# youshyee/CoSA

Measured on AMD Instinct MI355X. Metric: training images/sec at 448x448 ViT-B, higher is better.
Workload: dtype bf16; 1 GPU; VOC12 21-class, ViT-B/16 bf16, batch 16/GPU x 448x448, teacher 3 scales x 2 flips + student fwd/bwd + cam2mask x2 + 5 losses + AdamW + EMA; global_batch=16, parallelism=dp1, defer_groups=1, grid_policy=full grid

## Files before the change

### cosa_amd/csrc/gemm_kernels.hip

```cpp
#include "kernels.hpp"
#include "op16.hpp"
#include "c8.hpp"
#include "c4.hpp"
#include <cstdlib>

namespace cosa {
namespace {

typedef float f32x4 __attribute__((ext_vector_type(4)));

constexpr int BM = 128, BN = 128, BK = 64;
constexpr int TILE_BYTES = 128 * BK * 2;
constexpr int STAGE_BYTES = 2 * TILE_BYTES;
constexpr int CT_LD = 272;

enum { EPI_BIAS = 0, EPI_GELU = 1, EPI_RESIDUAL = 2 };

__device__ __forceinline__ float gelu_erf(float x)
{
    const float z = __builtin_fabsf(x) * 0.70710678118654752f;
    const float t = __builtin_amdgcn_rcpf(__builtin_fmaf(0.3275911f, z, 1.0f));
    float p = __builtin_fmaf(1.061405429f, t, -1.453152027f);
    p = __builtin_fmaf(p, t, 1.421413741f);
    p = __builtin_fmaf(p, t, -0.284496736f);
    p = __builtin_fmaf(p, t, 0.254829592f);
    p = p * t;
    const float e = __builtin_amdgcn_exp2f(-z * z * 1.4426950408889634f);
    const float erf_abs = __builtin_fmaf(-p, e, 1.0f);
    const float erfx = __builtin_copysignf(erf_abs, x);
    return 0.5f * x * (1.0f + erfx);
}

#define COSA_SPLIT_OPAQUE(a, b) asm volatile("" : "+v"(a), "+v"(b))

typedef __attribute__((address_space(3))) void lds_void;
typedef const __attribute__((address_space(1))) void gbl_void;

__device__ __forceinline__ void stage_tile(const op16 *__restrict__ src, int row0, int nrows, int ld, int k0,
                                           unsigned char *lds_tile, int wave, int lane)
{
#pragma unroll
    for (int i = 0; i < 4; i++) {
        const int q = wave * 4 + i;
        const int row = 8 * q + (lane >> 3);
        const int s = (lane & 7) ^ (row & 7);
        int grow = row0 + row;
        grow = grow < nrows ? grow : nrows - 1;
        const op16 *g = src + (size_t)grow * ld + k0 + s * 8;
        __builtin_amdgcn_global_load_lds((gbl_void *)g, (lds_void *)(lds_tile + q * 1024), 16, 0, 0);
    }
}

struct SplitGeom { int Kp; };
__device__ __forceinline__ int split_tile_x(int kt, int Kp) { return kt <= 2 * Kp ? kt : kt - 2 * Kp - 1; }
__device__ __forceinline__ int split_tile_w(int kt, int Kp) { return kt < Kp ? kt : (kt < 2 * Kp ? kt - Kp : (kt == 2 * Kp ? kt : kt - Kp - 1)); }

__device__ __forceinline__ bool c8_is_f8(int kt, int Kp) { return kt > Kp; }
__device__ __forceinline__ int c8_tile_x(int kt, int Kp) { return kt < Kp ? kt : (kt == Kp ? 2 * Kp : kt - 1); }
__device__ __forceinline__ int c8_tile_w(int kt, int Kp)
{
    const int Kh = Kp >> 1;
    return kt < Kp ? kt : (kt == Kp ? 2 * Kp : (kt <= Kp + Kh ? kt + Kh - 1 : kt - Kh - 1));
}
typedef int c8_i32x8 __attribute__((ext_vector_type(8)));
typedef int c8_i32x4 __attribute__((ext_vector_type(4)));
__device__ __forceinline__ c8_i32x8 c8_cat(op16x8 lo, op16x8 hi)
{
    return __builtin_shufflevector(__builtin_bit_cast(c8_i32x4, lo), __builtin_bit_cast(c8_i32x4, hi), 0, 1, 2, 3, 4, 5, 6, 7);
}
constexpr int kC8ScaleW = 0x7f7f7f7f;
constexpr int kC8ScaleX = 0x74747474;
#define COSA_MFMA_C8(a8, b8, c) __builtin_amdgcn_mfma_scale_f32_16x16x128_f8f6f4(a8, b8, c, 1, 1, 0, kC8ScaleW, 0, kC8ScaleX)

template <int OA, int OB>
__device__ __forceinline__ f32x4 mfma_c4(c8_i32x8 a4, c8_i32x8 b4, f32x4 c, int sa, int sb)
{
    return __builtin_amdgcn_mfma_scale_f32_16x16x128_f8f6f4(a4, b4, c, 4, 4, OA, sa, OB, sb);
}
__device__ __forceinline__ c8_i32x8 c4_op(op16x8 v)
{
    const c8_i32x4 t = __builtin_bit_cast(c8_i32x4, v);
    return (c8_i32x8){t[0], t[1], t[2], t[3], 0, 0, 0, 0};
}
__device__ __forceinline__ float c4_max4(float v)
{
    const unsigned u = __builtin_bit_cast(unsigned, v);
    const auto a = __builtin_amdgcn_permlane16_swap(u, u, false, false);
    const unsigned m = a[0] > a[1] ? a[0] : a[1];
    const auto b = __builtin_amdgcn_permlane32_swap(m, m, false, false);
    return __builtin_bit_cast(float, b[0] > b[1] ? b[0] : b[1]);
}
constexpr int kC4ScaleLds = 16384;
constexpr int kStageLdsC4 = 16384, kStageLds = 32768;

template <int EPI, int SPLIT = 0>
__global__ __launch_bounds__(256, 2) void gemm_bf16_kernel(const op16 *__restrict__ X, const op16 *__restrict__ W,
                                                          const op16 *__restrict__ bias, const float *__restrict__ R,
                                                          void *__restrict__ Yv, int M, int N, int K, int tiles_m, int tiles_n,
                                                          int ld, int ldy, void *__restrict__ Y2v, int tail_o0 = -1)
{
    static_assert(SPLIT < 3 || (SPLIT == 3 && EPI == EPI_RESIDUAL), "fp16c8 operands: residual epilogue (tail mode) only; fp16c4: not supported here");
    extern __shared__ __attribute__((aligned(16))) unsigned char smem[];
    const int tid = threadIdx.x, wave = tid >> 6, lane = tid & 63;
    int m0, n0;
    if (tail_o0 >= 0) {
        const int ntl = tiles_m * tiles_n, cq = ntl >> 3, cr = ntl & 7;
        const int o = tail_o0 + ((int)blockIdx.x >> 2), sub = blockIdx.x & 3;
        const int xcd = o & 7, idx = o >> 3;
        const int t = (xcd < cr ? xcd * (cq + 1) : cr * (cq + 1) + (xcd - cr) * cq) + idx;
        const int tm = t / tiles_n;
        m0 = tm * 256 + (sub >> 1) * BM;
        n0 = (t - tm * tiles_n) * 256 + (sub & 1) * BN;
        if (m0 >= M) return;
    } else {
        const int nwg = tiles_m * tiles_n;
        int wg = blockIdx.x;
        {
            const int q = nwg >> 3, r = nwg & 7, xcd = wg & 7, idx = wg >> 3;
            wg = (xcd < r ? xcd * (q + 1) : r * (q + 1) + (xcd - r) * q) + idx;
        }
        const int tm = wg / tiles_n, tn = wg - tm * tiles_n;
        m0 = tm * BM;
        n0 = tn * BN;
    }
    const int wr = wave >> 1, wc = wave & 1;

    f32x4 acc[4][4];
    const bool tail = tail_o0 >= 0;
#pragma unroll
    for (int i = 0; i < 4; i++)
#pragma unroll
        for (int j = 0; j < 4; j++) {
            acc[i][j] = (f32x4){0.f, 0.f, 0.f, 0.f};
            if (tail) {
                const int nl = (wave >> 1) * 64 + 16 * i + 4 * (lane >> 4), ml = (wave & 1) * 64 + 16 * j + (lane & 15);
                if (EPI == EPI_RESIDUAL) {
                    if (m0 + ml < M) acc[i][j] = *reinterpret_cast<const f32x4 *>(R + (size_t)(m0 + ml) * N + n0 + nl);
                } else {
#pragma unroll
                    for (int r = 0; r < 4; r++) acc[i][j][r] = (float)bias[n0 + nl + r];
                }
            }
        }

    const int Kp = K / BK;
    const int nk = SPLIT == 1 ? 3 * Kp + 1 : (SPLIT == 3 ? 2 * Kp + 1 : Kp);
    auto tile_x = [&](int kt) { return SPLIT == 1 ? split_tile_x(kt, Kp) : (SPLIT == 3 ? c8_tile_x(kt, Kp) : kt); };
    auto tile_w = [&](int kt) { return SPLIT == 1 ? split_tile_w(kt, Kp) : (SPLIT == 3 ? c8_tile_w(kt, Kp) : kt); };
    stage_tile(W, n0, N, ld, 0, smem, wave, lane);
    stage_tile(X, m0, M, ld, 0, smem + TILE_BYTES, wave, lane);
    asm volatile("s_waitcnt vmcnt(0)" ::: "memory");
    __syncthreads();

    const int frow = lane & 15, fq = lane >> 4;
    for (int kt = 0; kt < nk; kt++) {
        unsigned char *cur = smem + (kt & 1) * STAGE_BYTES;
        unsigned char *nxt = smem + ((kt + 1) & 1) * STAGE_BYTES;
        if (kt + 1 < nk) {
            stage_tile(W, n0, N, ld, tile_w(kt + 1) * BK, nxt, wave, lane);
            stage_tile(X, m0, M, ld, tile_x(kt + 1) * BK, nxt + TILE_BYTES, wave, lane);
        }
        const unsigned char *At = cur + (wr * 64) * 128;
        const unsigned char *Bt = cur + TILE_BYTES + (wc * 64) * 128;
        if (SPLIT == 3 && kt > Kp) {
            op16x8 a2[4][2], b2[4][2];
#pragma unroll
            for (int i = 0; i < 4; i++) {
                const int row = i * 16 + frow;
#pragma unroll
                for (int ks = 0; ks < 2; ks++) {
                    const int slot = ((fq + 4 * ks) ^ (row & 7)) << 4;
                    a2[i][ks] = *reinterpret_cast<const op16x8 *>(At + row * 128 + slot);
                    b2[i][ks] = *reinterpret_cast<const op16x8 *>(Bt + row * 128 + slot);
                }
            }
#pragma unroll
            for (int i = 0; i < 4; i++) {
                const c8_i32x8 a8 = c8_cat(a2[i][0], a2[i][1]);
#pragma unroll
                for (int j = 0; j < 4; j++) acc[i][j] = COSA_MFMA_C8(a8, c8_cat(b2[j][0], b2[j][1]), acc[i][j]);
            }
        } else
#pragma unroll
        for (int ks = 0; ks < 2; ks++) {
            op16x8 a[4], b[4];
#pragma unroll
            for (int i = 0; i < 4; i++) {
                const int row = i * 16 + frow;
                const int slot = ((fq + 4 * ks) ^ (row & 7)) << 4;
                a[i] = *reinterpret_cast<const op16x8 *>(At + row * 128 + slot);
                b[i] = *reinterpret_cast<const op16x8 *>(Bt + row * 128 + slot);
            }
#pragma unroll
            for (int i = 0; i < 4; i++)
#pragma unroll
                for (int j = 0; j < 4; j++)
                    acc[i][j] = COSA_MFMA_16x16x32(a[i], b[j], acc[i][j], 0, 0, 0);
        }
        asm volatile("s_waitcnt vmcnt(0)" ::: "memory");
        __syncthreads();
    }

    unsigned char *Ct = smem;
#pragma unroll
    for (int i = 0; i < 4; i++) {
        const int nl = wr * 64 + 16 * i + 4 * fq;
        float bv[4];
#pragma unroll
        for (int r = 0; r < 4; r++) bv[r] = (tail && EPI != EPI_RESIDUAL) ? 0.0f : (float)bias[n0 + nl + r];
#pragma unroll
        for (int j = 0; j < 4; j++) {
            const int ml = wc * 64 + 16 * j + frow;
            if (EPI == EPI_RESIDUAL) {
                f32x4 v;
#pragma unroll
                for (int r = 0; r < 4; r++) v[r] = acc[i][j][r] + bv[r];
                *reinterpret_cast<f32x4 *>(Ct + ml * (BN * 4 + 16) + nl * 4) = v;
            } else {
                op16x4 v, vlo;
#pragma unroll
                for (int r = 0; r < 4; r++) {
                    float t = acc[i][j][r] + bv[r];
                    if (SPLIT == 2) {
                        v[r] = (op16)t;
                        vlo[r] = (op16)gelu_erf(t);
                    } else {
                        if (EPI == EPI_GELU) t = gelu_erf(t);
                        if (SPLIT) asm volatile("" : "+v"(t));
                        v[r] = (op16)t;
                        if (SPLIT) vlo[r] = (op16)(t - (float)v[r]);
                    }
                }
                *reinterpret_cast<op16x4 *>(Ct + ml * CT_LD + nl * 2) = v;
                if (SPLIT) *reinterpret_cast<op16x4 *>(Ct + BM * CT_LD + ml * CT_LD + nl * 2) = vlo;
            }
        }
    }
    __syncthreads();
    if (EPI == EPI_RESIDUAL) {
        float *Y = static_cast<float *>(Yv);
#pragma unroll
        for (int c = tid; c < BM * 32; c += 256) {
            const int ml = c >> 5, s = c & 31;
            if (m0 + ml < M) {
                const f32x4 v = *reinterpret_cast<const f32x4 *>(Ct + ml * (BN * 4 + 16) + s * 16);
                const size_t o = (size_t)(m0 + ml) * N + n0 + s * 4;
                if (tail) {
                    *reinterpret_cast<f32x4 *>(Y + o) = v;
                } else {
                    const f32x4 rv = *reinterpret_cast<const f32x4 *>(R + o);
                    *reinterpret_cast<f32x4 *>(Y + o) = v + rv;
                }
            }
        }
    } else {
        op16 *Y = static_cast<op16 *>(Yv);
#pragma unroll
        for (int c = tid; c < BM * 16; c += 256) {
            const int ml = c >> 4, s = c & 15;
            if (m0 + ml < M) {
                *reinterpret_cast<uint4 *>(Y + (size_t)(m0 + ml) * ldy + n0 + s * 8) =
                    *reinterpret_cast<const uint4 *>(Ct + ml * CT_LD + s * 16);
                if (SPLIT == 1)
                    *reinterpret_cast<uint4 *>(Y + (size_t)(m0 + ml) * ldy + N + n0 + s * 8) =
                        *reinterpret_cast<const uint4 *>(Ct + BM * CT_LD + ml * CT_LD + s * 16);
                if (SPLIT == 2)
                    *reinterpret_cast<uint4 *>(static_cast<op16 *>(Y2v) + (size_t)(m0 + ml) * ldy + n0 + s * 8) =
                        *reinterpret_cast<const uint4 *>(Ct + BM * CT_LD + ml * CT_LD + s * 16);
            }
        }
    }
}


constexpr int V5_HALF = 16384;
constexpr int V5_BUF = 4 * V5_HALF;
constexpr size_t kLdsBytesV5 = 2 * V5_BUF;

#define V5_FENCE() __builtin_amdgcn_sched_barrier(0)
#define V5_BARRIER()                          \
    do {                                      \
        V5_FENCE();                           \
        __builtin_amdgcn_s_barrier();         \
        V5_FENCE();                           \
    } while (0)

typedef unsigned u32x2 __attribute__((ext_vector_type(2)));
typedef unsigned u32x4 __attribute__((ext_vector_type(4)));

template <int EPI, int SPLIT = 0, int FR = 4>
__global__ __launch_bounds__(512, 1) void gemm_bf16_v6_kernel(const op16 *__restrict__ X, const op16 *__restrict__ W,
                                                             const op16 *__restrict__ bias, const float *__restrict__ R,
                                                             void *__restrict__ Yv, int M, int N, int K, int tiles_m, int tiles_n,
                                                             unsigned long long *__restrict__ stamps, int ld, int ldy, void *__restrict__ Y2v, int ntiles_run,
                                                             const unsigned char *__restrict__ xsc, const unsigned char *__restrict__ wsc, unsigned char *__restrict__ ysc)
{
    if (stamps && threadIdx.x == 0) atomicMin(&stamps[2 * (blockIdx.x & 63)], __builtin_amdgcn_s_memrealtime());
    constexpr bool RES = EPI == EPI_RESIDUAL;
    constexpr int ES = RES ? 4 : 2;
    constexpr int FL = 0x00020000;
    static_assert(FR == 4 || (FR == 3 && SPLIT == 0), "FR: 16-feature fragments per wave and W half (tile width 64 FR)");
// ... 992 lines not shown
    for (int i = 0; i < PER; i++) {
        const float a = v[i].x - mean, c = v[i].y - mean, d = v[i].z - mean, e = v[i].w - mean;
        q += a * a + c * c + d * d + e * e;
    }
#pragma unroll
    for (int o = 32; o > 0; o >>= 1) q += __shfl_xor(q, o, 64);
    const float rstd = rsqrtf(q * (1.0f / D) + eps);
#pragma unroll
    for (int i = 0; i < PER; i++) {
        const int c0 = (lane + 64 * i) * 4;
        const op16x4 gg = *reinterpret_cast<const op16x4 *>(g + c0);
        const op16x4 bb = *reinterpret_cast<const op16x4 *>(b + c0);
        float o0 = (v[i].x - mean) * rstd * (float)gg[0] + (float)bb[0];
        float o1 = (v[i].y - mean) * rstd * (float)gg[1] + (float)bb[1];
        float o2 = (v[i].z - mean) * rstd * (float)gg[2] + (float)bb[2];
        float o3 = (v[i].w - mean) * rstd * (float)gg[3] + (float)bb[3];
        if (y) {
            op16x4 ov;
            ov[0] = (op16)o0; ov[1] = (op16)o1; ov[2] = (op16)o2; ov[3] = (op16)o3;
            *reinterpret_cast<op16x4 *>(y + (size_t)row * D + c0) = ov;
        }
        if (y32) *reinterpret_cast<float4 *>(y32 + (size_t)row * D + c0) = make_float4(o0, o1, o2, o3);
    }
}

}
}

using namespace cosa;

#if COSA_OP_F16
#define cosa_gemm_set_stamp_slot cosa_gemm_set_stamp_slot_f16
#define cosa_gemm_set_variant cosa_gemm_set_variant_f16
#define cosa_gemm_set_grid_policy cosa_gemm_set_grid_policy_f16
#define cosa_gemm_bf16 cosa_gemm_f16
#define cosa_gemm_bf16x3 cosa_gemm_f16x3
#define cosa_layernorm cosa_layernorm_f16
#define cosa_gemm_wgrad_bf16 cosa_gemm_wgrad_f16
#define cosa_conv3x3_dilated_wgrad cosa_conv3x3_dilated_wgrad_f16
#define cosa_conv3x3_dilated_nhwc cosa_conv3x3_dilated_nhwc_f16
#endif

#include <type_traits>

static size_t cosa_c4_scale_bytes_(int rows, int K) { return (size_t)((rows + 255) / 256) * (size_t)(K / 128) * 2048; }
static unsigned long long *g_gemm_stamp_slot = nullptr;
extern "C" void cosa_gemm_set_stamp_slot(void *slot) { g_gemm_stamp_slot = static_cast<unsigned long long *>(slot); }
namespace {
struct ClearSlot { ~ClearSlot() { g_gemm_stamp_slot = nullptr; } };
}

static int g_gemm_balanced_grid = 0;
static int g_gemm_variant = 0;
extern "C" void cosa_gemm_set_variant(int v) { g_gemm_variant = v; }
extern "C" void cosa_gemm_set_grid_policy(int balanced) { g_gemm_balanced_grid = balanced; }

template <auto Kernel>
static int max_dynamic_lds_once(int bytes)
{
    static bool done = false;
    if (!done) {
        COSA_HIP_CHECK(hipFuncSetAttribute((const void *)Kernel, hipFuncAttributeMaxDynamicSharedMemorySize, bytes));
        done = true;
    }
    return COSA_OK;
}

template <class F>
static int with_epilogue(int epilogue, F &&f)
{
    if (epilogue == EPI_BIAS) return f(std::integral_constant<int, EPI_BIAS>{});
    if (epilogue == EPI_GELU) return f(std::integral_constant<int, EPI_GELU>{});
    return f(std::integral_constant<int, EPI_RESIDUAL>{});
}

template <class... A>
static int check_gemm_args(const char *who, bool operands, const char *operands_what, int epilogue, const float *residual, bool shape_ok,
                           const char *shape_fmt, A... shape_args)
{
    COSA_REQUIRE(operands, "%s: %s", who, operands_what);
    COSA_REQUIRE(shape_ok, shape_fmt, shape_args...);
    COSA_REQUIRE(epilogue >= 0 && epilogue <= 2, "%s: unknown epilogue", who);
    COSA_REQUIRE(epilogue != EPI_RESIDUAL || residual, "%s: residual epilogue needs the residual pointer", who);
    return COSA_OK;
}

constexpr size_t kReach = 0x7fffffffull;
static bool fits_persistent(int M, int N, int ld) { return (size_t)(M + 256) * ld * 2 < kReach && (size_t)N * ld * 2 < kReach; }
static bool fits_persistent_x3(int M, int N, int ld) { return (size_t)(M + 256) * ld * 2 < kReach * 8 && (size_t)N * ld * 2 < kReach; }
static bool fits_panels(int N, int ld, int ldy) { return (size_t)256 * ld * 2 < kReach && (size_t)N * ld * 2 < kReach && (size_t)256 * ldy * 4 < kReach; }

constexpr int small_lds_bytes(int split)
{
    return ((split == 1 || split == 2) && 2 * BM * CT_LD > (int)kLdsBytes) ? 2 * BM * CT_LD : (int)kLdsBytes;
}


template <int EPI, int SPLIT>
static int launch_small(const op16 *x, const op16 *w, const op16 *b, const float *residual, void *Y, void *Y2, int M, int N, int K, int ld, int ldy,
                        hipStream_t st, int first_job = -1, int njobs = 0)
{
    constexpr int lds_bytes = small_lds_bytes(SPLIT);
    if (int rc = max_dynamic_lds_once<gemm_bf16_kernel<EPI, SPLIT>>(lds_bytes)) return rc;
    const bool tail = first_job >= 0;
    const int tiles_m = tail ? (M + 255) / 256 : (M + BM - 1) / BM, tiles_n = tail ? N / 256 : N / BN;
    hipLaunchKernelGGL((gemm_bf16_kernel<EPI, SPLIT>), dim3(tail ? 4 * njobs : tiles_m * tiles_n), dim3(256), lds_bytes, st, x, w, b, residual, Y,
                       M, N, K, tiles_m, tiles_n, ld ? ld : K, ldy ? ldy : N, Y2, first_job);
    COSA_LAUNCH_CHECK();
    return COSA_OK;
}

static int persistent_jobs(int ntiles)
{
    constexpr int tail_max = 48;
    const int rem = ntiles % 256, rounds_up = (ntiles + 255) / 256;
    if (ntiles > 256 && rem != 0 && rem <= tail_max && (256 - rem) * 10 > 256 * rounds_up) return ntiles - rem;
    return ntiles;
}

template <int EPI, int SPLIT = 0, int FR = 4>
static int launch_v6(const op16 *x, const op16 *w, const op16 *b, const float *residual, void *Y, int M, int N, int K, hipStream_t st,
                     int ld = 0, int ldy = 0, void *Y2 = nullptr, const unsigned char *xsc = nullptr, const unsigned char *wsc = nullptr,
                     unsigned char *ysc = nullptr)
{
    constexpr size_t lds_bytes = kLdsBytesV5 + (SPLIT == 4 ? kC4ScaleLds + kStageLdsC4 : kStageLds);
    if (int rc = max_dynamic_lds_once<gemm_bf16_v6_kernel<EPI, SPLIT, FR>>((int)lds_bytes)) return rc;
    const int tiles_m = (M + 255) / 256, tiles_n = N / (64 * FR);
    const int ntiles = tiles_m * tiles_n;
    const int grid = ntiles < 256 ? ntiles : 256;
    constexpr bool can_tail = FR == 4 && (SPLIT == 0 || SPLIT == 1 || (SPLIT == 3 && EPI == EPI_RESIDUAL));
    const int run = can_tail ? persistent_jobs(ntiles) : ntiles;
    const bool balanced = g_gemm_balanced_grid != 0;
    int grid_b = grid;
    if (balanced && run > 256 && M < 40000) {
        const int rounds = (run + 255) / 256;
        grid_b = ((run + rounds - 1) / rounds + 7) / 8 * 8;
        grid_b = grid_b > 256 ? 256 : grid_b;
    }
    hipLaunchKernelGGL((gemm_bf16_v6_kernel<EPI, SPLIT, FR>), dim3(grid_b), dim3(512), lds_bytes, st, x, w, b, residual, Y, M, N, K, tiles_m, tiles_n,
                       g_gemm_stamp_slot, ld ? ld : K, ldy ? ldy : N, Y2, run, xsc, wsc, ysc);
    g_gemm_stamp_slot = nullptr;
    COSA_LAUNCH_CHECK();
    if constexpr (can_tail) {
        if (run < ntiles) return launch_small<EPI, SPLIT>(x, w, b, residual, Y, nullptr, M, N, K, ld, ldy, st, run, ntiles - run);
    }
    return COSA_OK;
}

extern "C" int cosa_gemm_bf16(const void *X, const void *W, const void *bias, const float *residual, void *Y,
                              int M, int N, int K, int epilogue, void *stream)
{
    ClearSlot clear_slot_;
    const bool positive = M > 0 && N > 0 && K > 0;
    if (int rc = check_gemm_args("cosa_gemm_bf16", X && W && bias && Y, "null pointer", epilogue, residual, positive && N % BN == 0 && K % BK == 0,
                                 positive ? "cosa_gemm_bf16: N must be a multiple of 128 and K of 64 (got N=%d K=%d)" : "cosa_gemm_bf16: bad shape", N, K))
        return rc;
    hipStream_t st = as_stream(stream);
    const op16 *x = static_cast<const op16 *>(X), *w = static_cast<const op16 *>(W), *b = static_cast<const op16 *>(bias);
    const bool fits_v5 = N % 256 == 0 && M >= 256 && fits_persistent(M, N, K);
    constexpr int big_m = 4096;
    const bool fits_v6 = fits_v5 && K >= 128 && (epilogue != EPI_RESIDUAL || g_gemm_variant == 6 || g_gemm_variant == 9 || g_gemm_variant == 0);
    if (fits_v6 && N % 192 == 0 && (g_gemm_variant == 9 || (g_gemm_variant == 0 && M >= big_m))) {
        constexpr int wide_max = 48;
        const long tm = (M + 255) / 256, n4 = tm * (N / 256), n3 = tm * (N / 192);
        const double r4 = (n4 > 256 && n4 % 256 != 0 && n4 % 256 <= wide_max) ? (double)(n4 / 256) + 0.1 : (double)((n4 + 255) / 256);
        const double r3 = 0.78 * (double)((n3 + 255) / 256);
        if (g_gemm_variant == 9 || r3 < r4 - 0.05)
            return with_epilogue(epilogue, [&](auto e) { return launch_v6<decltype(e)::value, 0, 3>(x, w, b, residual, Y, M, N, K, st); });
    }
    if (fits_v6 && (g_gemm_variant == 6 || (g_gemm_variant == 0 && M >= big_m)))
        return with_epilogue(epilogue, [&](auto e) { return launch_v6<decltype(e)::value>(x, w, b, residual, Y, M, N, K, st); });
    return with_epilogue(epilogue, [&](auto e) { return launch_small<decltype(e)::value, 0>(x, w, b, residual, Y, nullptr, M, N, K, K, N, st); });
}

extern "C" int cosa_gemm_bf16x3(const void *Xs, const void *Ws, const void *zeros, const float *residual, void *Y,
                                int M, int N, int K, int epilogue, int ldy, void *stream)
// ... 208 lines not shown
```

### cosa_amd/nn_ops.py

```python
import contextlib
import ctypes
import math
import os
import time
import weakref

import torch
import torch.nn.functional as F
from torch.autograd import Function

from . import _C


_flops = {}


_reference_ops = None


def reference_op(name, what, *args, **kw):
    if _reference_ops is None:
        raise _C.CosaError(f"{what}: no HIP kernel covers this shape / dtype and cosa_amd has no second backend "
                           "(torch reference operators exist only in the test-suite: tests/torch_reference.py)")
    return _reference_ops[name](*args, **kw)
# ... 86 lines not shown
    def backward(ctx, dout):
        qkv, out, lse = ctx.saved_tensors
        H = ctx.H
        B, N, _ = qkv.shape
        dout = dout.contiguous()
        dqkv = torch.empty_like(qkv)
        L = _C.lib()
        ws = _C.workspace(L.cosa_attn_bwd_workspace_bytes(B, N, H), qkv.device, "attn_bwd")
        with _C.profiled("attn_bwd"):
            _C.check(L.cosa_attn_bwd(_C.ptr(qkv), _C.ptr(out), _C.ptr(dout), _C.ptr(lse), _C.ptr(dqkv), B, N, H, 64, 0.125,
                                     _C.ptr(ws), ws.numel(), _C.stream_ptr()), "cosa_attn_bwd")
        _flops["attn_bwd"] = _flops.get("attn_bwd", 0) + 10.0 * B * H * N * N * 64
        return dqkv, None


def attention(qkv, H):
    if qkv.dtype == torch.bfloat16:
        return FusedAttention.apply(qkv, H)
    return reference_op("attention", f"attention on {qkv.dtype} operands", qkv, H)


EPI_BIAS, EPI_GELU, EPI_RESIDUAL = 0, 1, 2


def gemm_bf16(x, w, b, epilogue=EPI_BIAS, residual=None, out=None):
    M, K = x.shape
    N = w.shape[0]
    dt = x.dtype
    assert w.dtype == dt and b.dtype == dt, "gemm: operands must share one 16-bit dtype"
    if out is None:
        out = torch.empty((M, N), device=x.device, dtype=torch.float32 if epilogue == EPI_RESIDUAL else dt)
    if gemm_stamps is not None and M >= 4096:
        nt = ((M + 255) // 256) * (N // 256) if N % 256 == 0 else 0
        rem, rounds_up = nt % 256, (nt + 255) // 256
        frac = (nt - rem) / nt if (nt > 256 and 0 < rem <= 48 and (256 - rem) * 10 > 256 * rounds_up) else 1.0
        _C.fn16("cosa_gemm_set_stamp_slot", dt)(gemm_stamps.next_slot(2.0 * M * N * K * frac))
    with _C.profiled("gemm_bf16"):
        _C.check(_C.fn16("cosa_gemm_bf16", dt)(_C.ptr(x), _C.ptr(w), _C.ptr(b), _C.ptr(residual), _C.ptr(out), M, N, K, epilogue,
                                               _C.stream_ptr()), "cosa_gemm_bf16")
    _flops["gemm_bf16"] = _flops.get("gemm_bf16", 0) + 2.0 * M * N * K
    return out


def conv3x3_dilated_tokens(tok, w16, B, h, w, dilation, relu=True):
    Cout, Cin = w16.shape[0], w16.shape[1]
    assert tok.dtype in (torch.bfloat16, torch.float16) and tok.dtype == w16.dtype
    assert tok.stride(2) == 1 and tok.shape[1] == h * w and tok.shape[2] == Cin
    ldx = tok.stride(1)
    img_rows = tok.stride(0) // ldx if B > 1 else h * w
    assert B == 1 or tok.stride(0) == img_rows * ldx
    wt = w16.permute(2, 3, 0, 1).reshape(9, Cout, Cin).contiguous()
    y = torch.empty((B * h * w, Cout), device=tok.device, dtype=tok.dtype)
    with _C.profiled("conv3x3"):
        _C.check(_C.fn16("cosa_conv3x3_dilated_nhwc", tok.dtype)(_C.ptr(tok), _C.ptr(wt), _C.ptr(y), B, h, w, Cin, Cout, int(dilation), img_rows, 0,
                                                    ldx, int(relu), _C.stream_ptr()), "cosa_conv3x3_dilated_nhwc")
    _flops["conv3x3"] = _flops.get("conv3x3", 0) + 2.0 * B * h * w * Cout * Cin * 9
    return y


def _token_view_geometry(tok, B, h, w):
    ldx = tok.stride(1)
    img_rows = tok.stride(0) // ldx if B > 1 else h * w
    assert tok.dtype == torch.bfloat16 and tok.stride(2) == 1 and tok.shape[1] == h * w
    assert B == 1 or tok.stride(0) == img_rows * ldx
    return ldx, img_rows


def conv3x3_dilated_wgrad(dy, tok, B, h, w, dilation):
# ... 999 lines not shown
```

### include/cosa_hip.h

```cpp
#ifndef COSA_HIP_H
#define COSA_HIP_H

#include <stddef.h>
#include <stdint.h>

#ifdef __cplusplus
extern "C" {
#endif

#define COSA_OK 0
#define COSA_EINVAL 1
#define COSA_EHIP 2
#define COSA_ERANGE 3
#define COSA_ENOMEM 4

int cosa_abi_version(void);
const char *cosa_last_error(void);

int cosa_denormalize_img(const float *img, float *out, int B, int H, int W, void *stream);

int cosa_cam_minmax_norm(float *cam, int BC, int HW, const float *active , void *stream);
int cosa_cam_minmax_norm_ws(float *cam, int BC, int HW, const float *active , void *workspace, void *stream);

int cosa_resize_bilinear(const float *src, float *dst, int planes, int H, int W, int OH, int OW, void *stream);
// ... 52 lines not shown
                              void *workspace, size_t workspace_bytes, void *stream);
int cosa_dense_energy_forward_prepared(const float *seg, const float *roi, const uint8_t *unlabel, float *AS, float *loss,
                                       int N, int K, int H, int W, float sigmargb, float sigmaxy,
                                       void *workspace, size_t workspace_bytes, void *stream);
int cosa_dense_energy_backward(const float *AS, const float *roi, const float *grad_out ,
                               float *grad_seg, int N, int K, int H, int W, void *stream);

size_t cosa_attn_workspace_bytes(int B, int N, int H);
int cosa_attn_prepare_vt(const void *qkv, int B, int N, int H, void *workspace, size_t workspace_bytes, void *stream);
int cosa_attn_fwd(const void *qkv, void *out, float *lse, int B, int N, int H, int head_dim, float scale,
                  int flags, uint64_t *stamps ,
                  void *workspace, size_t workspace_bytes, void *stream);

size_t cosa_attn_bwd_workspace_bytes(int B, int N, int H);
int cosa_attn_bwd(const void *qkv, const void *out, const void *dout, const float *lse, void *dqkv,
                  int B, int N, int H, int head_dim, float scale, void *workspace, size_t workspace_bytes, void *stream);

int cosa_gemm_bf16(const void *X, const void *W, const void *bias, const float *residual, void *Y,
                   int M, int N, int K, int epilogue, void *stream);
size_t cosa_gemm_wgrad_workspace_bytes(int M, int N, int K);
int cosa_gemm_wgrad_bf16(const void *dY, const void *X, float *dW, float *db, int M, int N, int K, int zero_first,
                         void *workspace, size_t workspace_bytes, void *stream);
typedef struct CosaWgradItem { const void *dY, *X; float *dW, *db; int N, K; } CosaWgradItem;
int cosa_gemm_wgrad_batched(const CosaWgradItem *items, int n_items, int M, void *stream);
size_t cosa_patch_wgrad_workspace_bytes(int M, int N, int K);
int cosa_patch_wgrad_bf16(const void *dY, const void *X, float *dW, float *db, int M, int N, int K, void *workspace, size_t workspace_bytes,
                          void *stream);
int cosa_conv3x3_dilated_nhwc(const void *X, const void *Wt, void *Y, int B, int h, int w, int Cin, int Cout, int dilation,
                              int img_rows, int row_off, int ldx, int relu, void *stream);
int cosa_conv3x3_dilated_wgrad(const void *dY, const void *X, float *dW9, int B, int h, int w, int Cin, int Cout, int dilation,
                               int img_rows, int row_off, int ldx, int zero_first, void *workspace, size_t workspace_bytes,
                               void *stream);
void cosa_gemm_set_variant(int v);
void cosa_gemm_set_grid_policy(int balanced);
void cosa_gemm_set_grid_policy_f16(int balanced);
void cosa_gemm_set_stamp_slot(void *slot);
int cosa_im2col_flip(const float *x, void *cols, int B, int C, int H, int W, int P, int flips, int dtype, void *stream);
int cosa_im2col_flip_c8_tokens(const float *x, void *rows, int B, int C, int H, int W, int P, int flips, int cls_rows, void *stream);
int cosa_im2col_flip_split_tokens(const float *x, void *rows, int B, int C, int H, int W, int P, int flips, int cls_rows, void *stream);
int cosa_im2col_flip_split_tokens_f16(const float *x, void *rows, int B, int C, int H, int W, int P, int flips, int cls_rows, void *stream);
int cosa_embed_finish(const void *tok, const void *cls, const void *pos, float *out, int B, int n, int D, int dtype, void *stream);
int cosa_head_gemm(const void *X, const void *W, float *Y, int M, int N, int K, int rows_per_img, long long img_stride,
                   int ldx, int dtype, int round_bf16, int ldy, int col0, void *stream);
int cosa_head_gemm_dgrad(const float *dY, const void *W, void *dX, int M, int N, int K, void *stream);
size_t cosa_head_gemm_wgrad_workspace(int M, int K);
int cosa_head_gemm_wgrad(const float *dY, const void *X, float *dW, void *workspace, int M, int N, int K, void *stream);
int cosa_layernorm(const float *x, const void *gamma, const void *beta, void *y_bf16, float *y_f32,
                   int rows, int dim, float eps, void *stream);
int cosa_broadcast_rows(const float *src, float *dst, int B, long long n, void *stream);
int cosa_pos_resize(const float *pe, const int *idx, const float *wgt, float *out, int P, int D, void *stream);
int cosa_gemm_bf16_dual_gelu(const void *X, const void *W, const void *bias, void *H, void *A, int M, int N, int K, void *stream);
int cosa_gelu_backward(const void *dA, const void *H, void *dH, long long n, void *stream);
size_t cosa_transpose_record_bytes(void);
int cosa_transpose_cast_batched(const void *records, int n, int total_tiles, void *stream);

int cosa_gemm_f16(const void *X, const void *W, const void *bias, const float *residual, void *Y,
                  int M, int N, int K, int epilogue, void *stream);
int cosa_gemm_wgrad_f16(const void *dY, const void *X, float *dW, float *db, int M, int N, int K, int zero_first,
                        void *workspace, size_t workspace_bytes, void *stream);
int cosa_layernorm_f16(const float *x, const void *gamma, const void *beta, void *y_f16, float *y_f32,
                       int rows, int dim, float eps, void *stream);
int cosa_conv3x3_dilated_nhwc_f16(const void *X, const void *Wt, void *Y, int B, int h, int w, int Cin, int Cout, int dilation,
                                  int img_rows, int row_off, int ldx, int relu, void *stream);
int cosa_conv3x3_dilated_wgrad_f16(const void *dY, const void *X, float *dW9, int B, int h, int w, int Cin, int Cout, int dilation,
                                   int img_rows, int row_off, int ldx, int zero_first, void *workspace, size_t workspace_bytes,
                                   void *stream);
void cosa_gemm_set_variant_f16(int v);
void cosa_gemm_set_stamp_slot_f16(void *slot);
size_t cosa_attn_workspace_bytes_f16(int B, int N, int H);
int cosa_attn_prepare_vt_f16(const void *qkv, int B, int N, int H, void *workspace, size_t workspace_bytes, void *stream);
int cosa_attn_fwd_f16(const void *qkv, void *out, float *lse, int B, int N, int H, int head_dim, float scale,
                      int flags, uint64_t *stamps, void *workspace, size_t workspace_bytes, void *stream);
size_t cosa_attn_bwd_workspace_bytes_f16(int B, int N, int H);
int cosa_attn_bwd_f16(const void *qkv, const void *out, const void *dout, const float *lse, void *dqkv,
                      int B, int N, int H, int head_dim, float scale, void *workspace, size_t workspace_bytes, void *stream);

int cosa_split_rows(const float *src, const float *bias, void *dst, int R, int K, long long src_ld, int ones, void *stream);
int cosa_layernorm_split(const float *x, const float *gamma, const float *beta, void *y_split, float *y_f32, int rows, int dim,
                         float eps, void *stream);
int cosa_gemm_bf16x3(const void *Xs, const void *Ws, const void *zeros, const float *residual, void *Y,
                     int M, int N, int K, int epilogue, int ldy, void *stream);
int cosa_attn_fwd_bf16x3(const void *qkv_split, void *out_split, float *lse, int B, int N, int H, int head_dim, float scale,
                         int ldq, int ldo, uint64_t *stamps , void *stream);
int cosa_split_rows_f16(const float *src, const float *bias, void *dst, int R, int K, long long src_ld, int ones, void *stream);
int cosa_layernorm_split_f16(const float *x, const float *gamma, const float *beta, void *y_split, float *y_f32, int rows, int dim,
                             float eps, void *stream);
int cosa_gemm_f16x3(const void *Xs, const void *Ws, const void *zeros, const float *residual, void *Y,
                    int M, int N, int K, int epilogue, int ldy, void *stream);
int cosa_attn_fwd_f16x3(const void *qkv_split, void *out_split, float *lse, int B, int N, int H, int head_dim, float scale,
                        int ldq, int ldo, uint64_t *stamps, void *stream);

int cosa_gemm_f32(const float *X, const float *W, const float *bias, const float *residual, float *Y, int M, int N, int K, int ldx, int ldw,
                  int ldr, int ldy, int epilogue, void *stream);
int cosa_conv3x3_dilated_f32(const float *tok, const float *Wt, float *Y, int B, int h, int w, int Cin, int Cout, int dilation, int img_rows,
                             int ldx, int relu, void *stream);
int cosa_attn_fwd_f32(const float *qkv, float *out, int B, int N, int H, int head_dim, float scale, int ldq, int ldo, void *stream);
int cosa_layernorm_f32out(const float *x, const float *gamma, const float *beta, float *y_f32, int rows, int dim, float eps, void *stream);
int cosa_im2col_flip_f32_tokens(const float *x, float *rows, int B, int C, int H, int W, int P, int flips, int cls_rows, void *stream);

int cosa_gemm_f64(const double *X, const void *W, const void *bias, const double *residual, double *Y, int M, int N, int K, int ldx, int ldw,
// ... 259 lines not shown
```

Baseline: 208.9 images/s.

## Add 64x64 tail tiles and a cost model for GEMM tail splitting

Templates the two-stage GEMM kernel on tile sides so tail launches can use 64x64 tiles, giving sixteen small workgroups per 256x256 leftover tile instead of four quarters. A calibrated cost model replaces the old fixed heuristic and picks among a full persistent round, 128 quarter tiles or 64 tiles, with a debug mode override and query hooks. The goal is to fill the GPU better on the wave-quantization tail of large GEMMs. The cost is hardcoded microsecond constants that may not fit other shapes, plus extra kernel instantiations.

```diff
diff --git a/cosa_amd/csrc/gemm_kernels.hip b/cosa_amd/csrc/gemm_kernels.hip
--- a/cosa_amd/csrc/gemm_kernels.hip
+++ b/cosa_amd/csrc/gemm_kernels.hip
@@ -36,12 +36,13 @@
 typedef __attribute__((address_space(3))) void lds_void;
 typedef const __attribute__((address_space(1))) void gbl_void;
 
+template <int ROWS = 128>
 __device__ __forceinline__ void stage_tile(const op16 *__restrict__ src, int row0, int nrows, int ld, int k0,
                                            unsigned char *lds_tile, int wave, int lane)
 {
 #pragma unroll
-    for (int i = 0; i < 4; i++) {
-        const int q = wave * 4 + i;
+    for (int i = 0; i < ROWS / 32; i++) {
+        const int q = wave * (ROWS / 32) + i;
         const int row = 8 * q + (lane >> 3);
         const int s = (lane & 7) ^ (row & 7);
         int grow = row0 + row;
@@ -93,24 +94,30 @@
 constexpr int kC4ScaleLds = 16384;
 constexpr int kStageLdsC4 = 16384, kStageLds = 32768;
 
-template <int EPI, int SPLIT = 0>
+template <int EPI, int SPLIT = 0, int TM = BM, int TN = BN>
 __global__ __launch_bounds__(256, 2) void gemm_bf16_kernel(const op16 *__restrict__ X, const op16 *__restrict__ W,
                                                           const op16 *__restrict__ bias, const float *__restrict__ R,
                                                           void *__restrict__ Yv, int M, int N, int K, int tiles_m, int tiles_n,
                                                           int ld, int ldy, void *__restrict__ Y2v, int tail_o0 = -1)
 {
     static_assert(SPLIT < 3 || (SPLIT == 3 && EPI == EPI_RESIDUAL), "fp16c8 operands: residual epilogue (tail mode) only; fp16c4: not supported here");
+    static_assert((TM == 128 || TM == 64) && (TN == 128 || TN == 64), "tile sides: 128 or 64");
+    static_assert(SPLIT != 3 || (TM == 128 && TN == 128), "fp16c8 operands: 128 x 128 quarters only");
+    constexpr int WM = TM / 2, WN = TN / 2, AI = WN / 16, AJ = WM / 16;
+    constexpr int W_BYTES = TN * BK * 2, STAGE = (TN + TM) * BK * 2;
+    constexpr int CT_LD = 2 * TN + 16, CT_LD32 = 4 * TN + 16;
     extern __shared__ __attribute__((aligned(16))) unsigned char smem[];
     const int tid = threadIdx.x, wave = tid >> 6, lane = tid & 63;
     int m0, n0;
     if (tail_o0 >= 0) {
+        constexpr int SUBS_N = 256 / TN, SUBS = (256 / TM) * SUBS_N;
         const int ntl = tiles_m * tiles_n, cq = ntl >> 3, cr = ntl & 7;
-        const int o = tail_o0 + ((int)blockIdx.x >> 2), sub = blockIdx.x & 3;
+        const int o = tail_o0 + (int)blockIdx.x / SUBS, sub = (int)blockIdx.x % SUBS;
         const int xcd = o & 7, idx = o >> 3;
         const int t = (xcd < cr ? xcd * (cq + 1) : cr * (cq + 1) + (xcd - cr) * cq) + idx;
         const int tm = t / tiles_n;
-        m0 = tm * 256 + (sub >> 1) * BM;
-        n0 = (t - tm * tiles_n) * 256 + (sub & 1) * BN;
+        m0 = tm * 256 + (sub / SUBS_N) * TM;
+        n0 = (t - tm * tiles_n) * 256 + (sub % SUBS_N) * TN;
         if (m0 >= M) return;
     } else {
         const int nwg = tiles_m * tiles_n;
@@ -120,20 +127,20 @@
             wg = (xcd < r ? xcd * (q + 1) : r * (q + 1) + (xcd - r) * q) + idx;
         }
         const int tm = wg / tiles_n, tn = wg - tm * tiles_n;
-        m0 = tm * BM;
-        n0 = tn * BN;
+        m0 = tm * TM;
+        n0 = tn * TN;
     }
     const int wr = wave >> 1, wc = wave & 1;
 
-    f32x4 acc[4][4];
+    f32x4 acc[AI][AJ];
     const bool tail = tail_o0 >= 0;
 #pragma unroll
-    for (int i = 0; i < 4; i++)
-#pragma unroll
-        for (int j = 0; j < 4; j++) {
+    for (int i = 0; i < AI; i++)
+#pragma unroll
+        for (int j = 0; j < AJ; j++) {
             acc[i][j] = (f32x4){0.f, 0.f, 0.f, 0.f};
             if (tail) {
-                const int nl = (wave >> 1) * 64 + 16 * i + 4 * (lane >> 4), ml = (wave & 1) * 64 + 16 * j + (lane & 15);
+                const int nl = (wave >> 1) * WN + 16 * i + 4 * (lane >> 4), ml = (wave & 1) * WM + 16 * j + (lane & 15);
                 if (EPI == EPI_RESIDUAL) {
                     if (m0 + ml < M) acc[i][j] = *reinterpret_cast<const f32x4 *>(R + (size_t)(m0 + ml) * N + n0 + nl);
                 } else {
@@ -147,25 +154,25 @@
     const int nk = SPLIT == 1 ? 3 * Kp + 1 : (SPLIT == 3 ? 2 * Kp + 1 : Kp);
     auto tile_x = [&](int kt) { return SPLIT == 1 ? split_tile_x(kt, Kp) : (SPLIT == 3 ? c8_tile_x(kt, Kp) : kt); };
     auto tile_w = [&](int kt) { return SPLIT == 1 ? split_tile_w(kt, Kp) : (SPLIT == 3 ? c8_tile_w(kt, Kp) : kt); };
-    stage_tile(W, n0, N, ld, 0, smem, wave, lane);
-    stage_tile(X, m0, M, ld, 0, smem + TILE_BYTES, wave, lane);
+    stage_tile<TN>(W, n0, N, ld, 0, smem, wave, lane);
+    stage_tile<TM>(X, m0, M, ld, 0, smem + W_BYTES, wave, lane);
     asm volatile("s_waitcnt vmcnt(0)" ::: "memory");
     __syncthreads();
 
     const int frow = lane & 15, fq = lane >> 4;
     for (int kt = 0; kt < nk; kt++) {
-        unsigned char *cur = smem + (kt & 1) * STAGE_BYTES;
-        unsigned char *nxt = smem + ((kt + 1) & 1) * STAGE_BYTES;
+        unsigned char *cur = smem + (kt & 1) * STAGE;
+        unsigned char *nxt = smem + ((kt + 1) & 1) * STAGE;
         if (kt + 1 < nk) {
-            stage_tile(W, n0, N, ld, tile_w(kt + 1) * BK, nxt, wave, lane);
-            stage_tile(X, m0, M, ld, tile_x(kt + 1) * BK, nxt + TILE_BYTES, wave, lane);
-        }
-        const unsigned char *At = cur + (wr * 64) * 128;
-        const unsigned char *Bt = cur + TILE_BYTES + (wc * 64) * 128;
+            stage_tile<TN>(W, n0, N, ld, tile_w(kt + 1) * BK, nxt, wave, lane);
+            stage_tile<TM>(X, m0, M, ld, tile_x(kt + 1) * BK, nxt + W_BYTES, wave, lane);
+        }
+        const unsigned char *At = cur + (wr * WN) * 128;
+        const unsigned char *Bt = cur + W_BYTES + (wc * WM) * 128;
         if (SPLIT == 3 && kt > Kp) {
-            op16x8 a2[4][2], b2[4][2];
-#pragma unroll
-            for (int i = 0; i < 4; i++) {
+            op16x8 a2[AI][2], b2[AJ][2];
+#pragma unroll
+            for (int i = 0; i < AI; i++) {
                 const int row = i * 16 + frow;
 #pragma unroll
                 for (int ks = 0; ks < 2; ks++) {
@@ -175,26 +182,26 @@
                 }
             }
 #pragma unroll
-            for (int i = 0; i < 4; i++) {
+            for (int i = 0; i < AI; i++) {
                 const c8_i32x8 a8 = c8_cat(a2[i][0], a2[i][1]);
 #pragma unroll
-                for (int j = 0; j < 4; j++) acc[i][j] = COSA_MFMA_C8(a8, c8_cat(b2[j][0], b2[j][1]), acc[i][j]);
+                for (int j = 0; j < AJ; j++) acc[i][j] = COSA_MFMA_C8(a8, c8_cat(b2[j][0], b2[j][1]), acc[i][j]);
             }
         } else
 #pragma unroll
         for (int ks = 0; ks < 2; ks++) {
-            op16x8 a[4], b[4];
-#pragma unroll
-            for (int i = 0; i < 4; i++) {
+            op16x8 a[AI], b[AJ];
+#pragma unroll
+            for (int i = 0; i < (AI > AJ ? AI : AJ); i++) {
                 const int row = i * 16 + frow;
                 const int slot = ((fq + 4 * ks) ^ (row & 7)) << 4;
-                a[i] = *reinterpret_cast<const op16x8 *>(At + row * 128 + slot);
-                b[i] = *reinterpret_cast<const op16x8 *>(Bt + row * 128 + slot);
+                if (i < AI) a[i] = *reinterpret_cast<const op16x8 *>(At + row * 128 + slot);
+                if (i < AJ) b[i] = *reinterpret_cast<const op16x8 *>(Bt + row * 128 + slot);
             }
 #pragma unroll
-            for (int i = 0; i < 4; i++)
-#pragma unroll
-                for (int j = 0; j < 4; j++)
+            for (int i = 0; i < AI; i++)
+#pragma unroll
+                for (int j = 0; j < AJ; j++)
                     acc[i][j] = COSA_MFMA_16x16x32(a[i], b[j], acc[i][j], 0, 0, 0);
         }
         asm volatile("s_waitcnt vmcnt(0)" ::: "memory");
@@ -203,19 +210,19 @@
 
     unsigned char *Ct = smem;
 #pragma unroll
-    for (int i = 0; i < 4; i++) {
-        const int nl = wr * 64 + 16 * i + 4 * fq;
+    for (int i = 0; i < AI; i++) {
+        const int nl = wr * WN + 16 * i + 4 * fq;
         float bv[4];
 #pragma unroll
         for (int r = 0; r < 4; r++) bv[r] = (tail && EPI != EPI_RESIDUAL) ? 0.0f : (float)bias[n0 + nl + r];
 #pragma unroll
-        for (int j = 0; j < 4; j++) {
-            const int ml = wc * 64 + 16 * j + frow;
+        for (int j = 0; j < AJ; j++) {
+            const int ml = wc * WM + 16 * j + frow;
             if (EPI == EPI_RESIDUAL) {
                 f32x4 v;
 #pragma unroll
                 for (int r = 0; r < 4; r++) v[r] = acc[i][j][r] + bv[r];
-                *reinterpret_cast<f32x4 *>(Ct + ml * (BN * 4 + 16) + nl * 4) = v;
+                *reinterpret_cast<f32x4 *>(Ct + ml * CT_LD32 + nl * 4) = v;
             } else {
                 op16x4 v, vlo;
 #pragma unroll
@@ -232,7 +239,7 @@
                     }
                 }
                 *reinterpret_cast<op16x4 *>(Ct + ml * CT_LD + nl * 2) = v;
-                if (SPLIT) *reinterpret_cast<op16x4 *>(Ct + BM * CT_LD + ml * CT_LD + nl * 2) = vlo;
+                if (SPLIT) *reinterpret_cast<op16x4 *>(Ct + TM * CT_LD + ml * CT_LD + nl * 2) = vlo;
             }
         }
     }
@@ -240,10 +247,10 @@
     if (EPI == EPI_RESIDUAL) {
         float *Y = static_cast<float *>(Yv);
 #pragma unroll
-        for (int c = tid; c < BM * 32; c += 256) {
-            const int ml = c >> 5, s = c & 31;
+        for (int c = tid; c < TM * (TN / 4); c += 256) {
+            const int ml = c / (TN / 4), s = c % (TN / 4);
             if (m0 + ml < M) {
-                const f32x4 v = *reinterpret_cast<const f32x4 *>(Ct + ml * (BN * 4 + 16) + s * 16);
+                const f32x4 v = *reinterpret_cast<const f32x4 *>(Ct + ml * CT_LD32 + s * 16);
                 const size_t o = (size_t)(m0 + ml) * N + n0 + s * 4;
                 if (tail) {
                     *reinterpret_cast<f32x4 *>(Y + o) = v;
@@ -256,17 +263,17 @@
     } else {
         op16 *Y = static_cast<op16 *>(Yv);
 #pragma unroll
-        for (int c = tid; c < BM * 16; c += 256) {
-            const int ml = c >> 4, s = c & 15;
+        for (int c = tid; c < TM * (TN / 8); c += 256) {
+            const int ml = c / (TN / 8), s = c % (TN / 8);
             if (m0 + ml < M) {
                 *reinterpret_cast<uint4 *>(Y + (size_t)(m0 + ml) * ldy + n0 + s * 8) =
                     *reinterpret_cast<const uint4 *>(Ct + ml * CT_LD + s * 16);
                 if (SPLIT == 1)
                     *reinterpret_cast<uint4 *>(Y + (size_t)(m0 + ml) * ldy + N + n0 + s * 8) =
-                        *reinterpret_cast<const uint4 *>(Ct + BM * CT_LD + ml * CT_LD + s * 16);
+                        *reinterpret_cast<const uint4 *>(Ct + TM * CT_LD + ml * CT_LD + s * 16);
                 if (SPLIT == 2)
                     *reinterpret_cast<uint4 *>(static_cast<op16 *>(Y2v) + (size_t)(m0 + ml) * ldy + n0 + s * 8) =
-                        *reinterpret_cast<const uint4 *>(Ct + BM * CT_LD + ml * CT_LD + s * 16);
+                        *reinterpret_cast<const uint4 *>(Ct + TM * CT_LD + ml * CT_LD + s * 16);
             }
         }
     }
@@ -1325,6 +1332,9 @@
 #if COSA_OP_F16
 #define cosa_gemm_set_stamp_slot cosa_gemm_set_stamp_slot_f16
 #define cosa_gemm_set_variant cosa_gemm_set_variant_f16
+#define cosa_gemm_set_tail_mode cosa_gemm_set_tail_mode_f16
+#define cosa_gemm_last_tail cosa_gemm_last_tail_f16
+#define cosa_gemm_tail_tile cosa_gemm_tail_tile_f16
 #define cosa_gemm_set_grid_policy cosa_gemm_set_grid_policy_f16
 #define cosa_gemm_bf16 cosa_gemm_f16
 #define cosa_gemm_bf16x3 cosa_gemm_f16x3
@@ -1383,32 +1393,65 @@
 static bool fits_persistent_x3(int M, int N, int ld) { return (size_t)(M + 256) * ld * 2 < kReach * 8 && (size_t)N * ld * 2 < kReach; }
 static bool fits_panels(int N, int ld, int ldy) { return (size_t)256 * ld * 2 < kReach && (size_t)N * ld * 2 < kReach && (size_t)256 * ldy * 4 < kReach; }
 
-constexpr int small_lds_bytes(int split)
-{
-    return ((split == 1 || split == 2) && 2 * BM * CT_LD > (int)kLdsBytes) ? 2 * BM * CT_LD : (int)kLdsBytes;
-}
-
-
-template <int EPI, int SPLIT>
+constexpr int small_lds_bytes(int split, int tm = BM, int tn = BN)
+{
+    const int stages = 2 * (tm + tn) * BK * 2, epi32 = tm * (4 * tn + 16), epi16 = ((split == 1 || split == 2) ? 2 : 1) * tm * (2 * tn + 16);
+    return stages > epi32 ? (stages > epi16 ? stages : epi16) : (epi32 > epi16 ? epi32 : epi16);
+}
+static_assert(small_lds_bytes(0) == (int)kLdsBytes && small_lds_bytes(1) == 2 * BM * CT_LD && small_lds_bytes(1, 64, 64) == 32768, "LDS of the two-stage kernel");
+
+static int g_gemm_tail_mode = 0;
+static int g_gemm_last_tail_jobs = 0, g_gemm_last_tail_tile = 0;
+extern "C" void cosa_gemm_set_tail_mode(int mode) { g_gemm_tail_mode = mode; }
+extern "C" void cosa_gemm_last_tail(int *jobs, int *tile)
+{
+    if (jobs) *jobs = g_gemm_last_tail_jobs;
+    if (tile) *tile = g_gemm_last_tail_tile;
+}
+
+template <int EPI, int SPLIT, int TM = BM, int TN = BN>
 static int launch_small(const op16 *x, const op16 *w, const op16 *b, const float *residual, void *Y, void *Y2, int M, int N, int K, int ld, int ldy,
                         hipStream_t st, int first_job = -1, int njobs = 0)
 {
-    constexpr int lds_bytes = small_lds_bytes(SPLIT);
-    if (int rc = max_dynamic_lds_once<gemm_bf16_kernel<EPI, SPLIT>>(lds_bytes)) return rc;
+    constexpr int lds_bytes = small_lds_bytes(SPLIT, TM, TN);
+    if (int rc = max_dynamic_lds_once<gemm_bf16_kernel<EPI, SPLIT, TM, TN>>(lds_bytes)) return rc;
     const bool tail = first_job >= 0;
+    COSA_REQUIRE(tail || (TM == BM && TN == BN), "two-stage GEMM kernel: tiles below 128 x 128 are for tail launches");
+    if (!tail) g_gemm_last_tail_jobs = g_gemm_last_tail_tile = 0;
     const int tiles_m = tail ? (M + 255) / 256 : (M + BM - 1) / BM, tiles_n = tail ? N / 256 : N / BN;
-    hipLaunchKernelGGL((gemm_bf16_kernel<EPI, SPLIT>), dim3(tail ? 4 * njobs : tiles_m * tiles_n), dim3(256), lds_bytes, st, x, w, b, residual, Y,
-                       M, N, K, tiles_m, tiles_n, ld ? ld : K, ldy ? ldy : N, Y2, first_job);
+    hipLaunchKernelGGL((gemm_bf16_kernel<EPI, SPLIT, TM, TN>), dim3(tail ? (256 / TM) * (256 / TN) * njobs : tiles_m * tiles_n), dim3(256), lds_bytes,
+                       st, x, w, b, residual, Y, M, N, K, tiles_m, tiles_n, ld ? ld : K, ldy ? ldy : N, Y2, first_job);
     COSA_LAUNCH_CHECK();
     return COSA_OK;
 }
 
-static int persistent_jobs(int ntiles)
-{
-    constexpr int tail_max = 48;
-    const int rem = ntiles % 256, rounds_up = (ntiles + 255) / 256;
-    if (ntiles > 256 && rem != 0 && rem <= tail_max && (256 - rem) * 10 > 256 * rounds_up) return ntiles - rem;
-    return ntiles;
+constexpr double kTailRoundTileUs = 0.78;
+constexpr double kTailRoundResidualUs = 21.0;
+constexpr double kTailQuarterUs = 4.0, kTailQuarterTileUs = 0.57;
+constexpr double kTailSmallUs = 1.2, kTailSmallTileUs = 0.475;
+constexpr double kTailSmallTile2Us = 0.51;
+constexpr double kTailMarginUs = 3.0;
+constexpr int kTailQuarterMaxJobs = 48, kTailSmallMaxJobs = 32;
+static int tail_choice(int ntiles, int nk, bool residual, bool small_ok)
+{
+    const int rem = ntiles % 256;
+    if (ntiles <= 256 || rem == 0) return 0;
+    const bool q_ok = rem <= kTailQuarterMaxJobs, s_ok = small_ok && rem <= kTailSmallMaxJobs;
+    if (g_gemm_tail_mode == 1) return 0;
+    if (g_gemm_tail_mode == 2) return q_ok ? 128 : 0;
+    if (g_gemm_tail_mode == 3) return s_ok ? 64 : 0;
+    double best = nk * kTailRoundTileUs + (residual ? kTailRoundResidualUs : 0.0) - kTailMarginUs;
+    int tile = 0;
+    const double quarters = kTailQuarterUs + nk * kTailQuarterTileUs, small = kTailSmallUs + nk * (rem <= 16 ? kTailSmallTileUs : kTailSmallTile2Us);
+    if (q_ok && quarters < best) best = quarters, tile = 128;
+    if (s_ok && small < best) tile = 64;
+    return tile;
+}
+
+extern "C" int cosa_gemm_tail_tile(int M, int N, int K, int epilogue)
+{
+    if (M <= 0 || N <= 0 || K <= 0 || N % 256 != 0) return 0;
+    return tail_choice((M + 255) / 256 * (N / 256), K / BK, epilogue == EPI_RESIDUAL, true);
 }
 
 template <int EPI, int SPLIT = 0, int FR = 4>
@@ -1422,7 +1465,12 @@
     const int ntiles = tiles_m * tiles_n;
     const int grid = ntiles < 256 ? ntiles : 256;
     constexpr bool can_tail = FR == 4 && (SPLIT == 0 || SPLIT == 1 || (SPLIT == 3 && EPI == EPI_RESIDUAL));
-    const int run = can_tail ? persistent_jobs(ntiles) : ntiles;
+    constexpr bool small_ok = SPLIT == 0 || SPLIT == 1;
+    const int nk = SPLIT == 1 ? 3 * (K / BK) + 1 : (SPLIT == 3 ? 2 * (K / BK) + 1 : K / BK);
+    const int tail_tile = can_tail ? tail_choice(ntiles, nk, EPI == EPI_RESIDUAL, small_ok) : 0;
+    const int run = tail_tile ? ntiles - ntiles % 256 : ntiles;
+    g_gemm_last_tail_jobs = ntiles - run;
+    g_gemm_last_tail_tile = tail_tile;
     const bool balanced = g_gemm_balanced_grid != 0;
     int grid_b = grid;
     if (balanced && run > 256 && M < 40000) {
@@ -1435,6 +1483,9 @@
     g_gemm_stamp_slot = nullptr;
     COSA_LAUNCH_CHECK();
     if constexpr (can_tail) {
+        if constexpr (small_ok) {
+            if (tail_tile == 64) return launch_small<EPI, SPLIT, 64, 64>(x, w, b, residual, Y, nullptr, M, N, K, ld, ldy, st, run, ntiles - run);
+        }
         if (run < ntiles) return launch_small<EPI, SPLIT>(x, w, b, residual, Y, nullptr, M, N, K, ld, ldy, st, run, ntiles - run);
     }
     return COSA_OK;
diff --git a/cosa_amd/nn_ops.py b/cosa_amd/nn_ops.py
--- a/cosa_amd/nn_ops.py
+++ b/cosa_amd/nn_ops.py
@@ -142,8 +142,7 @@
         out = torch.empty((M, N), device=x.device, dtype=torch.float32 if epilogue == EPI_RESIDUAL else dt)
     if gemm_stamps is not None and M >= 4096:
         nt = ((M + 255) // 256) * (N // 256) if N % 256 == 0 else 0
-        rem, rounds_up = nt % 256, (nt + 255) // 256
-        frac = (nt - rem) / nt if (nt > 256 and 0 < rem <= 48 and (256 - rem) * 10 > 256 * rounds_up) else 1.0
+        frac = (nt - nt % 256) / nt if nt and _C.fn16("cosa_gemm_tail_tile", dt)(M, N, K, epilogue) else 1.0
         _C.fn16("cosa_gemm_set_stamp_slot", dt)(gemm_stamps.next_slot(2.0 * M * N * K * frac))
     with _C.profiled("gemm_bf16"):
         _C.check(_C.fn16("cosa_gemm_bf16", dt)(_C.ptr(x), _C.ptr(w), _C.ptr(b), _C.ptr(residual), _C.ptr(out), M, N, K, epilogue,
diff --git a/include/cosa_hip.h b/include/cosa_hip.h
--- a/include/cosa_hip.h
+++ b/include/cosa_hip.h
@@ -108,6 +108,9 @@
                                int img_rows, int row_off, int ldx, int zero_first, void *workspace, size_t workspace_bytes,
                                void *stream);
 void cosa_gemm_set_variant(int v);
+void cosa_gemm_set_tail_mode(int mode);
+void cosa_gemm_last_tail(int *jobs, int *tile);
+int cosa_gemm_tail_tile(int M, int N, int K, int epilogue);
 void cosa_gemm_set_grid_policy(int balanced);
 void cosa_gemm_set_grid_policy_f16(int balanced);
 void cosa_gemm_set_stamp_slot(void *slot);
@@ -142,6 +145,9 @@
                                    int img_rows, int row_off, int ldx, int zero_first, void *workspace, size_t workspace_bytes,
                                    void *stream);
 void cosa_gemm_set_variant_f16(int v);
+void cosa_gemm_set_tail_mode_f16(int mode);
+void cosa_gemm_last_tail_f16(int *jobs, int *tile);
+int cosa_gemm_tail_tile_f16(int M, int N, int K, int epilogue);
 void cosa_gemm_set_stamp_slot_f16(void *slot);
 size_t cosa_attn_workspace_bytes_f16(int B, int N, int H);
 int cosa_attn_prepare_vt_f16(const void *qkv, int B, int N, int H, void *workspace, size_t workspace_bytes, void *stream);
```

After: 209.5 images/s (median of 6 runs). Within noise of the previous version (+0.3%).
